# talha-alam/ADAM-Dehaze

Hardware: AMD Instinct MI355X
Metric: images/sec CORUN-Complex fwd+bwd 512x1024 bs=8; PSNR vs CPU ref (higher is better)
Workload: dtype f32; 1 GPU; CORUN-Complex (HighIntensityDehazeModel base 96) train-mode fwd + L1 + bwd + Adam; per_gpu_batch=8, global_batch=8, height=512, width=1024, parallelism=dp1

## Files before the change

adam-dehaze_amd/csrc/bn_act.hip:

```cpp
#include "common.h"

__global__ __launch_bounds__(1024) void bn_finalize_kernel(const float* __restrict__ partials, int nblk, int NcP, int C,
                                                           double count, const float* __restrict__ gamma,
                                                           const float* __restrict__ beta, float eps, float momentum,
                                                           float* running_mean, float* running_var, float* scale,
                                                           float* shift, float* save_mean, float* save_invstd, int64_t* num_batches_tracked) {
    __shared__ double red[2][32][33];
    int c;
    double S, Q, mean, var;
    if (!bn_column_sums<4>(partials, nblk, NcP, C, red, c, S, Q)) return;
    bn_mean_var(S, Q, count, mean, var);
    bn_fold_channel(c, mean, var, count, gamma, beta, eps, momentum, running_mean, running_var, scale, shift, save_mean,
                    save_invstd, num_batches_tracked);
}

extern "C" int adh_bn_finalize(void* stream, const float* partials, int nblk, int NcP, int C, double count,
                               const float* gamma, const float* beta, float eps, float momentum, float* running_mean,
                               float* running_var, float* scale, float* shift, float* save_mean, float* save_invstd,
                               int64_t* num_batches_tracked) {
    if (!partials || !scale || !shift || nblk < 1 || C < 1 || NcP < C || count <= 0) return ADH_E_ARG;
    hipLaunchKernelGGL(bn_finalize_kernel, dim3(adh_ceil_div(C, 32)), dim3(1024), 0, (hipStream_t)stream, partials, nblk,
                       NcP, C, count, gamma, beta, eps, momentum, running_mean, running_var, scale, shift, save_mean,
                       save_invstd, num_batches_tracked);
    return adh_check_launch();
}

__global__ __launch_bounds__(1024) void bn_partial_sums_kernel(const float* __restrict__ partials, int nblk, int pitch, int C,
                                                               double count, double* __restrict__ sums) {
    __shared__ double red[2][32][33];
    int c;
    double S, Q;
    if (bn_column_sums<2>(partials, nblk, pitch, C, red, c, S, Q)) {
        sums[c] = S;
        sums[C + c] = Q;
    }
    if (blockIdx.x == 0 && threadIdx.x == 0) sums[2 * C] = count;
}

extern "C" int adh_bn_partial_sums(void* stream, const float* partials, int nblk, int pitch, int C, double count, double* sums) {
    if (!partials || !sums || nblk < 1 || C < 1 || pitch < C || count <= 0) return ADH_E_ARG;
    hipLaunchKernelGGL(bn_partial_sums_kernel, dim3(adh_ceil_div(C, 32)), dim3(1024), 0, (hipStream_t)stream, partials, nblk,
                       pitch, C, count, sums);
    return adh_check_launch();
}

__global__ void bn_finalize_sums_kernel(const double* __restrict__ sums, int C, const float* __restrict__ gamma,
                                        const float* __restrict__ beta, float eps, float momentum, float* running_mean,
                                        float* running_var, float* scale, float* shift, float* save_mean, float* save_invstd,
                                        int64_t* num_batches_tracked) {
    const int c = blockIdx.x * blockDim.x + threadIdx.x;
    if (c >= C) return;
    const double count = sums[2 * C];
    double mean, var;
    bn_mean_var(sums[c], sums[C + c], count, mean, var);
    bn_fold_channel(c, mean, var, count, gamma, beta, eps, momentum, running_mean, running_var, scale, shift, save_mean,
                    save_invstd, num_batches_tracked);
}

extern "C" int adh_bn_finalize_sums(void* stream, const double* sums, int C, const float* gamma, const float* beta, float eps,
                                    float momentum, float* running_mean, float* running_var, float* scale, float* shift,
                                    float* save_mean, float* save_invstd, int64_t* num_batches_tracked) {
    if (!sums || !scale || !shift || C < 1) return ADH_E_ARG;
    hipLaunchKernelGGL(bn_finalize_sums_kernel, dim3(adh_ceil_div(C, 128)), dim3(128), 0, (hipStream_t)stream, sums, C, gamma,
                       beta, eps, momentum, running_mean, running_var, scale, shift, save_mean, save_invstd, num_batches_tracked);
    return adh_check_launch();
// ... 156 lines not shown
                    const f32x4 gg = bn_masked_grad(g[u], act, mask_bits != nullptr, mb[u], mask_ss != nullptr, yy[u], msc, msh, o[u]);
                    sg += gg;
                    sgx += gg * ((yy[u] - mu) * is);
                }
            }
        }
    }
    bn_block_fold(red, sg, sgx, CQ, R, c, C, partials);
  }
}

extern "C" int adh_bn_bwd_reduce(void* stream, const float* g_out, int g_cs, const float* out, int out_cs, int act,
                                 const float* y, int y_cs, const float* mean, const float* invstd, float* partials,
                                 int64_t P, int C, const float* mask_ss, const uint8_t* mask_bits) {
    if (!g_out || !y || !mean || !invstd || !partials || P < 1 || C < 4 || (C & 3) || C > 4096) return ADH_E_ARG;
    if (act == ADH_ACT_RELU && !out && !mask_ss && !mask_bits) return ADH_E_ARG;
    if (mask_bits && (((C / 4) & 1) || act != ADH_ACT_RELU)) return ADH_E_ARG;
    if (!adh_act_host_valid(act) || (act > ADH_ACT_RELU && !mask_ss)) return ADH_E_ARG;
    hipLaunchKernelGGL(bn_bwd_reduce_kernel, dim3(adh_bn_bwd_num_blocks(P, C)), dim3(256), 0, (hipStream_t)stream, g_out,
                       g_cs, out, out_cs, act, y, y_cs, mean, invstd, partials, P, C, mask_ss, mask_bits);
    return adh_check_launch();
}

__global__ __launch_bounds__(1024) void bn_bwd_finalize_kernel(const float* __restrict__ partials, int nblk, int pitch, int C,
                                                               double count, const float* gamma, const float* invstd,
                                                               float* dgamma, float* dbeta, int accumulate, float* coef,
                                                               int centered) {
    __shared__ double red[2][32][33];
    int c;
    double S, Q;
    if (!bn_column_sums<4>(partials, nblk, pitch, C, red, c, S, Q)) return;
    if (centered) Q *= (double)invstd[c];
    bn_bwd_coef_channel(c, C, S, Q, S, Q, count, gamma, invstd, dgamma, dbeta, accumulate, coef);
}

extern "C" int adh_bn_bwd_finalize(void* stream, const float* partials, int nblk, int C, double count,
                                   const float* gamma, const float* invstd, float* dgamma, float* dbeta, int accumulate,
                                   float* coef) {
    if (!partials || !invstd || !coef || nblk < 1 || C < 1 || count <= 0) return ADH_E_ARG;
    hipLaunchKernelGGL(bn_bwd_finalize_kernel, dim3(adh_ceil_div(C, 32)), dim3(1024), 0, (hipStream_t)stream, partials,
                       nblk, C, C, count, gamma, invstd, dgamma, dbeta, accumulate, coef, 0);
    return adh_check_launch();
}

extern "C" int adh_bn_bwd_finalize_centered(void* stream, const float* partials, int nblk, int pitch, int C, double count,
                                            const float* gamma, const float* invstd, float* dgamma, float* dbeta,
                                            int accumulate, float* coef) {
    if (!partials || !invstd || !coef || nblk < 1 || C < 1 || pitch < C || count <= 0) return ADH_E_ARG;
    hipLaunchKernelGGL(bn_bwd_finalize_kernel, dim3(adh_ceil_div(C, 32)), dim3(1024), 0, (hipStream_t)stream, partials,
                       nblk, pitch, C, count, gamma, invstd, dgamma, dbeta, accumulate, coef, 1);
    return adh_check_launch();
}

__global__ __launch_bounds__(256) void bn_bwd_apply_kernel(const float* __restrict__ g_out, int g_cs,
                                                           const float* __restrict__ out, int out_cs, int act,
                                                           const float* __restrict__ y, int y_cs,
                                                           const float* __restrict__ mean,
                                                           const float* __restrict__ invstd,
                                                           const float* __restrict__ coef, int training,
                                                           float* __restrict__ g_y, int gy_cs, float* __restrict__ g_res,
                                                           int gres_cs, int64_t P, int C, const float* __restrict__ mask_ss,
                                                           const uint8_t* __restrict__ mask_bits) {
    const int CQ = C / 4;
    int64_t p, pstep;
    int c;
    adh_stream_decode(CQ, p, pstep, c);
    const f32x4 k0 = *reinterpret_cast<const f32x4*>(coef + c);
    f32x4 mg = {0.f, 0.f, 0.f, 0.f}, kx = mg, mu = mg, msc = mg, msh = mg;
    if (mask_ss) {
        msc = *reinterpret_cast<const f32x4*>(mask_ss + c);
        msh = *reinterpret_cast<const f32x4*>(mask_ss + C + c);
    }
    if (training) {
// ... 60 lines not shown
```

adam-dehaze_amd/csrc/bn_stream.h:

```cpp
#pragma once

__host__ __device__ static inline bool adh_act_valid(int act) {
    return act == ADH_ACT_NONE || act == ADH_ACT_RELU || act == ADH_ACT_RELU6 || act == ADH_ACT_HARDSWISH ||
           act == ADH_ACT_HARDSIGMOID;
}
static inline bool adh_act_host_valid(int act) { return adh_act_valid(act); }
__device__ __forceinline__ float adh_act_fwd(int act, float z) {
    switch (act) {
        case ADH_ACT_RELU: return fmaxf(z, 0.f);
        case ADH_ACT_RELU6: return fminf(fmaxf(z, 0.f), 6.f);
        case ADH_ACT_HARDSWISH: return z * fminf(fmaxf(z + 3.f, 0.f), 6.f) / 6.f;
        case ADH_ACT_HARDSIGMOID: return fminf(fmaxf(z + 3.f, 0.f), 6.f) / 6.f;
        default: return z;
    }
}
__device__ __forceinline__ float adh_act_bwd(int act, float z, float g) {
    switch (act) {
        case ADH_ACT_RELU: return z > 0.f ? g : 0.f;
        case ADH_ACT_RELU6: return (z > 0.f && z < 6.f) ? g : 0.f;
        case ADH_ACT_HARDSWISH: return z <= -3.f ? 0.f : (z < 3.f ? g * (z / 3.f + 0.5f) : g);
        case ADH_ACT_HARDSIGMOID: return (z > -3.f && z < 3.f) ? g / 6.f : 0.f;
        default: return g;
    }
}
// ... 37 lines not shown
    CQ = (C - cbase < 1024 ? C - cbase : 1024) / 4;
    R = 256 / CQ;
    const int cq = threadIdx.x % CQ;
    prow = threadIdx.x / CQ;
    c = cbase + cq * 4;
}
__device__ __forceinline__ void bn_block_fold(f32x4 (&red)[2][256], const f32x4& a, const f32x4& b, int CQ, int R, int c, int C,
                                              float* partials) {
    red[0][threadIdx.x] = a;
    red[1][threadIdx.x] = b;
    __syncthreads();
    if (threadIdx.x < CQ) {
        f32x4 sa = {0.f, 0.f, 0.f, 0.f}, sb = {0.f, 0.f, 0.f, 0.f};
        for (int r = 0; r < R; ++r) {
            sa += red[0][r * CQ + threadIdx.x];
            sb += red[1][r * CQ + threadIdx.x];
        }
        *reinterpret_cast<f32x4*>(partials + ((size_t)blockIdx.x * 2 + 0) * C + c) = sa;
        *reinterpret_cast<f32x4*>(partials + ((size_t)blockIdx.x * 2 + 1) * C + c) = sb;
    }
    __syncthreads();
}

template <int CHAINS>
__device__ __forceinline__ bool bn_column_sums(const float* __restrict__ partials, int nblk, int pitch, int C,
                                               double (&red)[2][32][33], int& c, double& S, double& Q) {
    static_assert(CHAINS == 2 || CHAINS == 4, "two or four chains");
    const int cx = threadIdx.x & 31, ry = threadIdx.x >> 5;
    c = blockIdx.x * 32 + cx;
    double s[CHAINS] = {}, q[CHAINS] = {};
    if (c < C) {
        int b = ry;
        for (; b + 32 * (CHAINS - 1) < nblk; b += 32 * CHAINS) {
#pragma unroll
            for (int k = 0; k < CHAINS; ++k) {
                s[k] += (double)partials[((size_t)(b + 32 * k) * 2 + 0) * pitch + c];
                q[k] += (double)partials[((size_t)(b + 32 * k) * 2 + 1) * pitch + c];
            }
        }
        for (; b < nblk; b += 32) {
            s[0] += (double)partials[((size_t)b * 2 + 0) * pitch + c];
            q[0] += (double)partials[((size_t)b * 2 + 1) * pitch + c];
        }
    }
    if constexpr (CHAINS == 4) {
        red[0][ry][cx] = (s[0] + s[1]) + (s[2] + s[3]);
        red[1][ry][cx] = (q[0] + q[1]) + (q[2] + q[3]);
    } else {
        red[0][ry][cx] = s[0] + s[1];
        red[1][ry][cx] = q[0] + q[1];
    }
    __syncthreads();
    if (ry != 0 || c >= C) return false;
    S = 0.0;
    Q = 0.0;
    for (int r = 0; r < 32; ++r) {
        S += red[0][r][cx];
        Q += red[1][r][cx];
    }
    return true;
}

__device__ __forceinline__ void bn_mean_var(double S, double Q, double count, double& mean, double& var) {
    mean = S / count;
    var = Q / count - mean * mean;
    if (var < 0.0) var = 0.0;
}

__device__ __forceinline__ void bn_fold_channel(int c, double mean, double var, double count, const float* __restrict__ gamma,
                                                const float* __restrict__ beta, float eps, float momentum, float* running_mean,
                                                float* running_var, float* scale, float* shift, float* save_mean,
                                                float* save_invstd, int64_t* num_batches_tracked) {
    const double invstd = 1.0 / sqrt(var + (double)eps);
    const float gm = gamma ? gamma[c] : 1.f;
    const float bt = beta ? beta[c] : 0.f;
    scale[c] = (float)(gm * invstd);
    shift[c] = (float)(bt - mean * gm * invstd);
    if (save_mean) save_mean[c] = (float)mean;
    if (save_invstd) save_invstd[c] = (float)invstd;
    if (running_mean) running_mean[c] = (1.f - momentum) * running_mean[c] + momentum * (float)mean;
    if (running_var) {
// ... 16 lines not shown
```

adam-dehaze_amd/csrc/cbam.hip:

```cpp
#include "common.h"

#ifndef POOL_PPB
#define POOL_PPB 512
#endif
#ifndef CBAM_SCALE_MAXBLK
#define CBAM_SCALE_MAXBLK 65536
#endif
#ifndef CBAM_ROW_MAXBLK
#define CBAM_ROW_MAXBLK 2048
#endif

extern "C" int adh_cbam_pool_num_blocks(int HW) { return adh_ceil_div(HW, POOL_PPB); }

__global__ __launch_bounds__(256) void cbam_pool_partial_kernel(const float* __restrict__ x, int x_cs, int HW, int C,
                                                                float* __restrict__ partial,
                                                                int32_t* __restrict__ partial_idx, int nblk) {
    __shared__ f32x4 rs[256];
    __shared__ f32x4 rm[256];
    __shared__ int ri[256][4];
    const int n = blockIdx.y, blk = blockIdx.x;
    const int CQ = C / 4;
    const int R = 256 / CQ;
    const int cq = threadIdx.x % CQ, prow = threadIdx.x / CQ;
    const int c = cq * 4;
// ... 300 lines not shown
                            __builtin_nontemporal_load(reinterpret_cast<const f32x4*>(gn + (size_t)p * g_cs + q * 4));
            s += (v[0] + v[1]) + (v[2] + v[3]);
        }
#pragma unroll
        for (int o = 4; o > 0; o >>= 1) s += __shfl_xor(s, o, 64);
        if (sub == 0) {
            const float a = sa[(size_t)n * HW + p];
            gsa_pre[(size_t)n * HW + p] = s * a * (1.f - a);
        }
    }
}

extern "C" int adh_cbam_bwd_a(void* stream, const float* g, int g_cs, const float* x, int x_cs, const float* ca,
                              const float* sa, int N, int HW, int C, float* gsa_pre) {
    if (!g || !x || !ca || !sa || !gsa_pre || N < 1 || HW < 1 || C < 4 || (C & 3)) return ADH_E_ARG;
    const int blocks = adh_min_i(adh_ceil_div(HW, 32), CBAM_ROW_MAXBLK);
    hipLaunchKernelGGL(cbam_bwd_a_kernel, dim3(blocks, N), dim3(256), 0, (hipStream_t)stream, g, g_cs, x, x_cs, ca, sa, HW,
                       C, gsa_pre);
    return adh_check_launch();
}

extern "C" int adh_cbam_bwd_b_num_blocks(int N, int H, int W) { return adh_ceil_div((int64_t)N * H * W, 256); }

__global__ __launch_bounds__(256) void cbam_bwd_b_kernel(const float* __restrict__ gsa_pre,
                                                         const float* __restrict__ smap, const float* __restrict__ wsp,
                                                         int N, int H, int W, float* __restrict__ gsmap,
                                                         float* __restrict__ dwsp_partial) {
    __shared__ float s_w[98];
    __shared__ float s_acc[4][98];
    if (threadIdx.x < 98) s_w[threadIdx.x] = wsp[threadIdx.x];
    __syncthreads();
    const int64_t total = (int64_t)N * H * W;
    const int64_t idx = (int64_t)blockIdx.x * 256 + threadIdx.x;
    const bool valid = idx < total;
    int n = 0, y = 0, xx = 0;
    if (valid) {
        xx = (int)(idx % W);
        const int64_t r = idx / W;
        y = (int)(r % H);
        n = (int)(r / H);
    }
    const float* gp = gsa_pre + (size_t)n * H * W;
    const float* sm = smap + (size_t)n * H * W * 2;
    const float gs_here = valid ? gp[(size_t)y * W + xx] : 0.f;
    float g0 = 0.f, g1 = 0.f;
    const int wave = threadIdx.x >> 6, lane = threadIdx.x & 63;
    for (int ky = 0; ky < 7; ++ky) {
        for (int kx = 0; kx < 7; ++kx) {
            const int oy = y - ky + 3, ox = xx - kx + 3;
            if (valid && oy >= 0 && oy < H && ox >= 0 && ox < W) {
                const float go = gp[(size_t)oy * W + ox];
                g0 += go * s_w[ky * 7 + kx];
                g1 += go * s_w[49 + ky * 7 + kx];
            }
            const int iy = y + ky - 3, ix = xx + kx - 3;
            float a0 = 0.f, a1 = 0.f;
            if (valid && iy >= 0 && iy < H && ix >= 0 && ix < W) {
                const float* q = sm + ((size_t)iy * W + ix) * 2;
                a0 = q[0] * gs_here;
                a1 = q[1] * gs_here;
            }
            a0 = wave_sum(a0);
            a1 = wave_sum(a1);
            if (lane == 0) {
                s_acc[wave][ky * 7 + kx] = a0;
                s_acc[wave][49 + ky * 7 + kx] = a1;
            }
        }
    }
    if (valid) {
        gsmap[idx * 2 + 0] = g0;
        gsmap[idx * 2 + 1] = g1;
    }
    __syncthreads();
    if (threadIdx.x < 98)
        dwsp_partial[(size_t)blockIdx.x * 98 + threadIdx.x] =
            (s_acc[0][threadIdx.x] + s_acc[1][threadIdx.x]) + (s_acc[2][threadIdx.x] + s_acc[3][threadIdx.x]);
}

__global__ __launch_bounds__(256) void cbam_dwsp_final_kernel(const float* __restrict__ partial, int nblk, float* dwsp,
                                                              int accumulate) {
    __shared__ double red[256];
    const int o = blockIdx.x;
    double s = 0.0;
    for (int b = threadIdx.x; b < nblk; b += 256) s += (double)partial[(size_t)b * 98 + o];
    red[threadIdx.x] = s;
    __syncthreads();
    for (int st = 128; st > 0; st >>= 1) {
        if (threadIdx.x < st) red[threadIdx.x] += red[threadIdx.x + st];
        __syncthreads();
    }
    if (threadIdx.x == 0) dwsp[o] = accumulate ? dwsp[o] + (float)red[0] : (float)red[0];
}

extern "C" int adh_cbam_bwd_b(void* stream, const float* gsa_pre, const float* smap, const float* wsp, int N, int H,
                              int W, float* gsmap, float* dwsp_partial, int nblk, float* dwsp, int accumulate) {
    if (!gsa_pre || !smap || !wsp || !gsmap || !dwsp_partial || !dwsp) return ADH_E_ARG;
    if (nblk != adh_cbam_bwd_b_num_blocks(N, H, W)) return ADH_E_ARG;
    hipStream_t s = (hipStream_t)stream;
    hipLaunchKernelGGL(cbam_bwd_b_kernel, dim3(nblk), dim3(256), 0, s, gsa_pre, smap, wsp, N, H, W, gsmap, dwsp_partial);
// ... 226 lines not shown
```

adam-dehaze_amd/csrc/conv_wgrad.hip:

```cpp
#include "common.h"
#include <cstdlib>

#define WG_TW 32

template <int T, int TN>
__global__ __launch_bounds__(512, 2) void conv_wgrad_kernel(const adh_conv_desc d, const ConvGeom g, float* slab,
                                                            int ntiles, int KP, int nco_groups) {
    extern __shared__ __attribute__((aligned(16))) float smem[];
    constexpr int BN = 32 * TN;
    constexpr int PER = (T * TN + 3) / 4;
    const int XP = g.xp;
    const int buf_floats = g.npx * XP + 32 + g.TH * WG_TW * BN;

    const int tid = threadIdx.x;
    const int lane = tid & 63;
    const int wave = __builtin_amdgcn_readfirstlane(tid >> 6);
    const bool loader = wave >= 4;
    const int l31 = lane & 31;
    const int h = lane >> 5;

    const int ci_tile = blockIdx.x / nco_groups;
    const int co_grp = blockIdx.x - ci_tile * nco_groups;
    const int ci0 = ci_tile * 32;
    const int co0 = co_grp * BN;
// ... 456 lines not shown
        if (2 * bytes <= 160 * 1024 || TH == 1) break;
        TH >>= 1;
    }
    g->TH = TH;
    g->npxp = g->npx;
    g->tiles_x = adh_ceil_div(d->VW, WG_TW);
    g->tiles_y = adh_ceil_div(d->VH, TH);
    g->KC = 32;
    g->KQ_log2 = 3;
    g->KQtot = 0;
    g->xp = xp;
    return ADH_OK;
}

template <int T, int TN>
static void launch_wgrad(hipStream_t s, const adh_conv_desc* d, const ConvGeom& g, float* slab, int nsplit, int KP) {
    const int ntiles = g.tiles_x * g.tiles_y * d->N;
    const int nco_groups = d->NcP / (32 * TN);
    const int lds = 2 * (g.npx * g.xp * 4 + 128 + g.TH * WG_TW * 32 * TN * 4);
    dim3 grid((KP / 32) * nco_groups, nsplit, (d->KH * d->KW) / T);
    (void)hipFuncSetAttribute(reinterpret_cast<const void*>(&conv_wgrad_kernel<T, TN>),
                              hipFuncAttributeMaxDynamicSharedMemorySize, 160 * 1024);
    hipLaunchKernelGGL((conv_wgrad_kernel<T, TN>), grid, dim3(512), lds, s, *d, g, slab, ntiles, KP, nco_groups);
}

static int wgrad_pick_tn(int NcP, int T) {
    const int t = NcP / 32;
    for (int tn = 4; tn >= 1; --tn)
        if (t % tn == 0 && (T * tn + 3) / 4 <= 12) return tn;
    return 1;
}

struct WrPlan {
    int KH, KW, rev, TN;
    WrArgs a;
};

static int wgrad_rows_plan(const adh_conv_desc* d, int nsplit, WrPlan plan[4]) {
    if (d->VW % 32 != 0 || d->VH % WR_TH != 0) return 0;
    if (d->Cin % 32 != 0 || d->Cout % 4 != 0 || d->NcP != adh_round_up(d->Cout, 32)) return 0;
    if (d->in_cstride % 4 != 0 || d->out_cstride % 4 != 0) return 0;
    if (d->in_sy != d->in_sx || d->dstep_y != d->dstep_x || d->out_sy != d->out_sx) return 0;
    if ((d->VH - 1) * d->out_sy + d->out_oy >= d->OH || (d->VW - 1) * d->out_sx + d->out_ox >= d->OW) return 0;
    if ((int64_t)(d->IH + 8) * d->IW * d->in_cstride * 4 >= (int64_t)1 << 31) return 0;
    if ((int64_t)d->OH * d->OW * d->out_cstride * 4 >= (int64_t)1 << 31) return 0;
    const int t = d->NcP / 32;
// ... 113 lines not shown
        WrPlan plan[4];
        const int np = wgrad_rows_plan(d, nsplit, plan);
        if (np && wgrad_rows_instantiated(plan[0])) {
            for (int i = 0; i < np; ++i) {
                const int rc = dispatch_wgrad_rows((hipStream_t)stream, d, plan[i], slab);
                if (rc) return rc;
            }
            return ADH_OK;
        }
    }
    const int Ttot = d->KH * d->KW;
    int T;
    if (Ttot == 9 || Ttot == 16 || Ttot == 4 || Ttot == 1) T = Ttot;
    else if (Ttot == 49 || Ttot == 14) T = 7;
    else return ADH_E_UNSUPPORTED;
    const bool packed = (d->dstep_x == 4 && d->Cin == 8 && d->in_sx == 1);
    const int TN = wgrad_pick_tn(d->NcP, T);
    ConvGeom g;
    int rc = wgrad_geometry(d, &g, TN, packed ? 8 : 32);
    if (rc) return rc;
    if ((d->VH - 1) * d->out_sy + d->out_oy >= d->OH || (d->VW - 1) * d->out_sx + d->out_ox >= d->OW) return ADH_E_ARG;
    const int KP = adh_round_up(d->Cin, 32);
    hipStream_t s = (hipStream_t)stream;
#define WG_CASE(t, tn) \
    if (T == t && TN == tn) { launch_wgrad<t, tn>(s, d, g, slab, nsplit, KP); return adh_check_launch(); }
    WG_CASE(9, 4) WG_CASE(9, 3) WG_CASE(9, 2) WG_CASE(9, 1)
    WG_CASE(16, 3) WG_CASE(16, 2) WG_CASE(16, 1)
    WG_CASE(4, 4) WG_CASE(4, 3) WG_CASE(4, 2) WG_CASE(4, 1)
    WG_CASE(7, 4) WG_CASE(7, 3) WG_CASE(7, 2) WG_CASE(7, 1)
    WG_CASE(1, 4) WG_CASE(1, 3) WG_CASE(1, 2) WG_CASE(1, 1)
#undef WG_CASE
    return ADH_E_UNSUPPORTED;
}
```

adam-dehaze_amd/csrc/conv_wgrad_small.hip:

```cpp
#include "common.h"

typedef float f32x4s __attribute__((ext_vector_type(4)));

template <int XC, int GC, int CIB>
__global__ __launch_bounds__(256) void conv_wgrad_small_kernel(const adh_conv_desc d, int tiles_x, int tiles_y, int ntiles,
                                                               float* __restrict__ slab, int KP, int NcP) {
    extern __shared__ __attribute__((aligned(16))) float lds[];
    constexpr int XS_F = 6 * 66 * XC + 16;
    float* const xs = lds;
    float* const gs = lds + XS_F;

    const int tid = threadIdx.x;
    const int lane = tid & 63;
    const int wave = tid >> 6;
    const int i16 = lane & 15, kk = lane >> 4;

    f32x4s acc[9 * CIB];
#pragma unroll
    for (int t = 0; t < 9 * CIB; ++t) acc[t] = f32x4s{0.f, 0.f, 0.f, 0.f};

    for (int tile = blockIdx.x; tile < ntiles; tile += gridDim.x) {
        int r = tile;
        const int tx = r % tiles_x;
        r /= tiles_x;
        const int ty = r % tiles_y;
        const int n = r / tiles_y;
        const int y0 = ty * 4, x0 = tx * 64;
        const float* xin = d.in + (int64_t)n * d.IH * d.IW * XC;
        const float* gin = d.out + (int64_t)n * d.VH * d.VW * GC;
        __syncthreads();
        constexpr int XQ = XC / 4;
        for (int i = tid; i < 6 * 66 * XQ; i += 256) {
            const int px = i / XQ, q = i - px * XQ;
            const int row = px / 66, col = px - row * 66;
            const int iy = y0 - 1 + row, ix = x0 - 1 + col;
            f32x4s v = {0.f, 0.f, 0.f, 0.f};
            if (iy >= 0 && iy < d.IH && ix >= 0 && ix < d.IW)
                v = *reinterpret_cast<const f32x4s*>(xin + ((int64_t)iy * d.IW + ix) * XC + q * 4);
            *reinterpret_cast<f32x4s*>(xs + px * XC + q * 4) = v;
        }
        constexpr int GQ = GC / 4;
        for (int i = tid; i < 4 * 64 * GQ; i += 256) {
            const int px = i / GQ, q = i - px * GQ;
            const int row = px >> 6, col = px & 63;
            const int gy = y0 + row, gx = x0 + col;
            f32x4s v = {0.f, 0.f, 0.f, 0.f};
            if (gy < d.VH && gx < d.VW) v = *reinterpret_cast<const f32x4s*>(gin + ((int64_t)gy * d.VW + gx) * GC + q * 4);
            *reinterpret_cast<f32x4s*>(gs + px * GC + q * 4) = v;
        }
        if (tid < 16) {
            xs[6 * 66 * XC + tid] = 0.f;
            gs[4 * 64 * GC + tid] = 0.f;
        }
        __syncthreads();
        const float* gl = gs + (wave * 64 + kk) * GC + i16;
        const float* xl = xs + (wave * 66 + kk) * XC + i16;
#pragma unroll 2
        for (int kg = 0; kg < 16; ++kg) {
            const float b = gl[kg * 4 * GC];
#pragma unroll
            for (int dy = 0; dy < 3; ++dy)
#pragma unroll
                for (int dx = 0; dx < 3; ++dx)
#pragma unroll
                    for (int cb = 0; cb < CIB; ++cb) {
                        const float a = xl[(dy * 66 + kg * 4 + dx) * XC + cb * 16];
                        acc[(dy * 3 + dx) * CIB + cb] =
                            __builtin_amdgcn_mfma_f32_16x16x4f32(a, b, acc[(dy * 3 + dx) * CIB + cb], 0, 0, 0);
                    }
        }
    }

    float* red = lds;
#pragma unroll 1
    for (int w = 1; w < 4; ++w) {
        __syncthreads();
        if (wave == w) {
// ... 26 lines not shown
                                                                float* __restrict__ slab, int KP, int NcP) {
    extern __shared__ __attribute__((aligned(16))) float lds[];
    constexpr int CJB = XC / 16;
    constexpr int RT = (9 * COUT + 15) / 16;
    constexpr int GS_F = 6 * 66 * GC + 16;
    float* const gs = lds;
    float* const xs = lds + GS_F;
    const int tid = threadIdx.x;
    const int lane = tid & 63;
    const int wave = tid >> 6;
    const int i16 = lane & 15, kk = lane >> 4;
    int aoff[RT];
#pragma unroll
    for (int t = 0; t < RT; ++t) {
        const int rI = adh_min_i(t * 16 + i16, 9 * COUT - 1);
        const int tap = rI / COUT, co = rI - tap * COUT;
        const int dy = tap / 3, dx = tap - dy * 3;
        aoff[t] = ((2 - dy) * 66 + (2 - dx)) * GC + co;
    }
    f32x4s acc[RT * CJB];
#pragma unroll
    for (int t = 0; t < RT * CJB; ++t) acc[t] = f32x4s{0.f, 0.f, 0.f, 0.f};

    for (int tile = blockIdx.x; tile < ntiles; tile += gridDim.x) {
        int r = tile;
        const int tx = r % tiles_x;
        r /= tiles_x;
        const int ty = r % tiles_y;
        const int n = r / tiles_y;
        const int y0 = ty * 4, x0 = tx * 64;
        const float* xin = d.in + (int64_t)n * d.IH * d.IW * XC;
        const float* gin = d.out + (int64_t)n * d.VH * d.VW * GC;
        __syncthreads();
        constexpr int GQ = GC / 4;
        for (int i = tid; i < 6 * 66 * GQ; i += 256) {
            const int px = i / GQ, q = i - px * GQ;
            const int row = px / 66, col = px - row * 66;
            const int gy = y0 - 1 + row, gx = x0 - 1 + col;
            f32x4s v = {0.f, 0.f, 0.f, 0.f};
            if (gy >= 0 && gy < d.VH && gx >= 0 && gx < d.VW) v = *reinterpret_cast<const f32x4s*>(gin + ((int64_t)gy * d.VW + gx) * GC + q * 4);
            *reinterpret_cast<f32x4s*>(gs + px * GC + q * 4) = v;
        }
        constexpr int XQ = XC / 4;
        for (int i = tid; i < 4 * 64 * XQ; i += 256) {
            const int px = i / XQ, q = i - px * XQ;
            const int row = px >> 6, col = px & 63;
            const int iy = y0 + row, ix = x0 + col;
            f32x4s v = {0.f, 0.f, 0.f, 0.f};
            if (iy < d.IH && ix < d.IW) v = *reinterpret_cast<const f32x4s*>(xin + ((int64_t)iy * d.IW + ix) * XC + q * 4);
            *reinterpret_cast<f32x4s*>(xs + px * XC + q * 4) = v;
        }
        if (tid < 16) gs[6 * 66 * GC + tid] = 0.f;
        __syncthreads();
        const float* gl = gs + (wave * 66 + kk) * GC;
        const float* xl = xs + (wave * 64 + kk) * XC + i16;
#pragma unroll 4
        for (int kg = 0; kg < 16; ++kg) {
            float a[RT], b[CJB];
#pragma unroll
            for (int t = 0; t < RT; ++t) a[t] = gl[kg * 4 * GC + aoff[t]];
#pragma unroll
            for (int c = 0; c < CJB; ++c) b[c] = xl[kg * 4 * XC + c * 16];
#pragma unroll
            for (int t = 0; t < RT; ++t)
#pragma unroll
                for (int c = 0; c < CJB; ++c)
                    acc[t * CJB + c] = __builtin_amdgcn_mfma_f32_16x16x4f32(a[t], b[c], acc[t * CJB + c], 0, 0, 0);
        }
    }
    float* red = lds;
#pragma unroll 1
    for (int w = 1; w < 4; ++w) {
        __syncthreads();
        if (wave == w) {
#pragma unroll
            for (int t = 0; t < RT * CJB; ++t) *reinterpret_cast<f32x4s*>(red + (t * 64 + lane) * 4) = acc[t];
// ... 71 lines not shown
```

adam-dehaze_amd/csrc/densenet.hip:

```cpp
#include "common.h"

#define SS_PPB 512
#define SS_UNROLL 4

extern "C" int adh_bn_slice_stats_num_blocks(int64_t P, int C) {
    (void)C;
    return P < 1 ? ADH_E_ARG : adh_ceil_div(P, SS_PPB);
}

__global__ __launch_bounds__(256) void bn_slice_stats_kernel(const float* __restrict__ x, int x_cs, int64_t P, int C,
                                                             float* __restrict__ partials) {
    __shared__ f32x4 red[2][256];
    for (int cbase = 0; cbase < C; cbase += 1024) {
        int CQ, R, prow, c;
        bn_group_decode(C, cbase, CQ, R, prow, c);
        f32x4 s = {0.f, 0.f, 0.f, 0.f}, q = s;
        if (prow < R) {
            const int64_t p0 = (int64_t)blockIdx.x * SS_PPB;
            const int64_t p1 = p0 + SS_PPB < P ? p0 + SS_PPB : P;
            for (int64_t p = p0 + prow; p < p1; p += SS_UNROLL * R) {
                f32x4 v[SS_UNROLL];
#pragma unroll
                for (int u = 0; u < SS_UNROLL; ++u) {
                    const int64_t r = p + u * R < p1 ? p + u * R : p;
                    v[u] = __builtin_nontemporal_load(reinterpret_cast<const f32x4*>(x + r * x_cs + c));
                }
#pragma unroll
                for (int u = 0; u < SS_UNROLL; ++u)
                    if (p + u * R < p1) {
                        s += v[u];
                        q += v[u] * v[u];
                    }
            }
        }
        bn_block_fold(red, s, q, CQ, R, c, C, partials);
    }
}

extern "C" int adh_bn_slice_stats(void* stream, const float* x, int x_cs, int64_t P, int C, float* partials) {
    if (!x || !partials || P < 1 || C < 4 || (C & 3) || C > 4096 || x_cs < C || (x_cs & 3)) return ADH_E_ARG;
    hipLaunchKernelGGL(bn_slice_stats_kernel, dim3(adh_bn_slice_stats_num_blocks(P, C)), dim3(256), 0, (hipStream_t)stream, x,
                       x_cs, P, C, partials);
    return adh_check_launch();
}

__global__ __launch_bounds__(1024) void bn_slice_moments_kernel(const float* __restrict__ partials, int nblk, int pitch, int C,
                                                                double count, double* __restrict__ mean,
                                                                double* __restrict__ var) {
    __shared__ double red[2][32][33];
    int c;
    double S, Q, m, v;
    if (!bn_column_sums<2>(partials, nblk, pitch, C, red, c, S, Q)) return;
    bn_mean_var(S, Q, count, m, v);
    mean[c] = m;
    var[c] = v;
}

extern "C" int adh_bn_slice_moments(void* stream, const float* partials, int nblk, int pitch, int C, double count, double* mean,
                                    double* var) {
    if (!partials || !mean || !var || nblk < 1 || C < 1 || pitch < C || count <= 0) return ADH_E_ARG;
    hipLaunchKernelGGL(bn_slice_moments_kernel, dim3(adh_ceil_div(C, 32)), dim3(1024), 0, (hipStream_t)stream, partials, nblk,
                       pitch, C, count, mean, var);
    return adh_check_launch();
}

__global__ void bn_fold_moments_kernel(int C, const double* __restrict__ mean, const double* __restrict__ var, double count,
                                       const float* __restrict__ gamma, const float* __restrict__ beta, float eps,
                                       float momentum, float* running_mean, float* running_var, float* scale, float* shift,
                                       float* save_mean, float* save_invstd, int64_t* num_batches_tracked) {
    const int c = blockIdx.x * blockDim.x + threadIdx.x;
    if (c >= C) return;
    bn_fold_channel(c, mean[c], var[c], count, gamma, beta, eps, momentum, running_mean, running_var, scale, shift, save_mean,
                    save_invstd, num_batches_tracked);
}

extern "C" int adh_bn_fold_moments(void* stream, int C, const double* mean, const double* var, double count, const float* gamma,
                                   const float* beta, float eps, float momentum, float* running_mean, float* running_var,
                                   float* scale, float* shift, float* save_mean, float* save_invstd,
                                   int64_t* num_batches_tracked) {
    if (C < 1 || !mean || !var || !scale || !shift || count <= 0) return ADH_E_ARG;
    hipLaunchKernelGGL(bn_fold_moments_kernel, dim3(adh_ceil_div(C, 256)), dim3(256), 0, (hipStream_t)stream, C, mean, var, count,
                       gamma, beta, eps, momentum, running_mean, running_var, scale, shift, save_mean, save_invstd,
                       num_batches_tracked);
    return adh_check_launch();
}
// ... 87 lines not shown
```

Baseline: 40.43 images/sec.

## Retune BN column reduction, prefetch wgrad tiles, add 1x1 few-output wgrad kernel

BN column-sum kernels now use 8 channels per block with 256 threads and a batched, unrolled load loop, which gives more blocks and more loads in flight per thread. The small-channel wgrad kernels prefetch the next tile into registers while computing the current one, overlapping global loads with compute at the cost of extra registers. A dedicated 1x1 wgrad kernel handles layers with at most 32 inputs and 4 outputs. The CBAM backward replaces per-tap wave reductions with LDS staging and a per-row fold, which adds shared memory and barriers.

New measurement: 40.68 images/sec (median of 6 runs). No clear change (+0.6%).

```diff
diff --git a/adam-dehaze_amd/csrc/bn_act.hip b/adam-dehaze_amd/csrc/bn_act.hip
--- a/adam-dehaze_amd/csrc/bn_act.hip
+++ b/adam-dehaze_amd/csrc/bn_act.hip
@@ -1,11 +1,12 @@
 #include "common.h"
 
-__global__ __launch_bounds__(1024) void bn_finalize_kernel(const float* __restrict__ partials, int nblk, int NcP, int C,
+__global__ __launch_bounds__(BN_COLS_THREADS) void bn_finalize_kernel(const float* __restrict__ partials,
+                                                                    int nblk, int NcP, int C,
                                                            double count, const float* __restrict__ gamma,
                                                            const float* __restrict__ beta, float eps, float momentum,
                                                            float* running_mean, float* running_var, float* scale,
                                                            float* shift, float* save_mean, float* save_invstd, int64_t* num_batches_tracked) {
-    __shared__ double red[2][32][33];
+    __shared__ BnColsLds red;
     int c;
     double S, Q, mean, var;
     if (!bn_column_sums<4>(partials, nblk, NcP, C, red, c, S, Q)) return;
@@ -19,15 +20,16 @@
                                float* running_var, float* scale, float* shift, float* save_mean, float* save_invstd,
                                int64_t* num_batches_tracked) {
     if (!partials || !scale || !shift || nblk < 1 || C < 1 || NcP < C || count <= 0) return ADH_E_ARG;
-    hipLaunchKernelGGL(bn_finalize_kernel, dim3(adh_ceil_div(C, 32)), dim3(1024), 0, (hipStream_t)stream, partials, nblk,
-                       NcP, C, count, gamma, beta, eps, momentum, running_mean, running_var, scale, shift, save_mean,
-                       save_invstd, num_batches_tracked);
-    return adh_check_launch();
-}
-
-__global__ __launch_bounds__(1024) void bn_partial_sums_kernel(const float* __restrict__ partials, int nblk, int pitch, int C,
+    hipLaunchKernelGGL(bn_finalize_kernel, dim3(adh_ceil_div(C, BN_COLS_CH)), dim3(BN_COLS_THREADS), 0, (hipStream_t)stream,
+                       partials, nblk, NcP, C, count, gamma, beta, eps, momentum, running_mean, running_var, scale, shift,
+                       save_mean, save_invstd, num_batches_tracked);
+    return adh_check_launch();
+}
+
+__global__ __launch_bounds__(BN_COLS_THREADS) void bn_partial_sums_kernel(const float* __restrict__ partials,
+                                                                        int nblk, int pitch, int C,
                                                                double count, double* __restrict__ sums) {
-    __shared__ double red[2][32][33];
+    __shared__ BnColsLds red;
     int c;
     double S, Q;
     if (bn_column_sums<2>(partials, nblk, pitch, C, red, c, S, Q)) {
@@ -39,8 +41,8 @@
 
 extern "C" int adh_bn_partial_sums(void* stream, const float* partials, int nblk, int pitch, int C, double count, double* sums) {
     if (!partials || !sums || nblk < 1 || C < 1 || pitch < C || count <= 0) return ADH_E_ARG;
-    hipLaunchKernelGGL(bn_partial_sums_kernel, dim3(adh_ceil_div(C, 32)), dim3(1024), 0, (hipStream_t)stream, partials, nblk,
-                       pitch, C, count, sums);
+    hipLaunchKernelGGL(bn_partial_sums_kernel, dim3(adh_ceil_div(C, BN_COLS_CH)), dim3(BN_COLS_THREADS), 0, (hipStream_t)stream,
+                       partials, nblk, pitch, C, count, sums);
     return adh_check_launch();
 }
 
@@ -243,11 +245,12 @@
     return adh_check_launch();
 }
 
-__global__ __launch_bounds__(1024) void bn_bwd_finalize_kernel(const float* __restrict__ partials, int nblk, int pitch, int C,
+__global__ __launch_bounds__(BN_COLS_THREADS) void bn_bwd_finalize_kernel(const float* __restrict__ partials,
+                                                                        int nblk, int pitch, int C,
                                                                double count, const float* gamma, const float* invstd,
                                                                float* dgamma, float* dbeta, int accumulate, float* coef,
                                                                int centered) {
-    __shared__ double red[2][32][33];
+    __shared__ BnColsLds red;
     int c;
     double S, Q;
     if (!bn_column_sums<4>(partials, nblk, pitch, C, red, c, S, Q)) return;
@@ -259,8 +262,8 @@
                                    const float* gamma, const float* invstd, float* dgamma, float* dbeta, int accumulate,
                                    float* coef) {
     if (!partials || !invstd || !coef || nblk < 1 || C < 1 || count <= 0) return ADH_E_ARG;
-    hipLaunchKernelGGL(bn_bwd_finalize_kernel, dim3(adh_ceil_div(C, 32)), dim3(1024), 0, (hipStream_t)stream, partials,
-                       nblk, C, C, count, gamma, invstd, dgamma, dbeta, accumulate, coef, 0);
+    hipLaunchKernelGGL(bn_bwd_finalize_kernel, dim3(adh_ceil_div(C, BN_COLS_CH)), dim3(BN_COLS_THREADS), 0, (hipStream_t)stream,
+                       partials, nblk, C, C, count, gamma, invstd, dgamma, dbeta, accumulate, coef, 0);
     return adh_check_launch();
 }
 
@@ -268,8 +271,8 @@
                                             const float* gamma, const float* invstd, float* dgamma, float* dbeta,
                                             int accumulate, float* coef) {
     if (!partials || !invstd || !coef || nblk < 1 || C < 1 || pitch < C || count <= 0) return ADH_E_ARG;
-    hipLaunchKernelGGL(bn_bwd_finalize_kernel, dim3(adh_ceil_div(C, 32)), dim3(1024), 0, (hipStream_t)stream, partials,
-                       nblk, pitch, C, count, gamma, invstd, dgamma, dbeta, accumulate, coef, 1);
+    hipLaunchKernelGGL(bn_bwd_finalize_kernel, dim3(adh_ceil_div(C, BN_COLS_CH)), dim3(BN_COLS_THREADS), 0, (hipStream_t)stream,
+                       partials, nblk, pitch, C, count, gamma, invstd, dgamma, dbeta, accumulate, coef, 1);
     return adh_check_launch();
 }
 
diff --git a/adam-dehaze_amd/csrc/bn_stream.h b/adam-dehaze_amd/csrc/bn_stream.h
--- a/adam-dehaze_amd/csrc/bn_stream.h
+++ b/adam-dehaze_amd/csrc/bn_stream.h
@@ -83,15 +83,46 @@
     __syncthreads();
 }
 
+#define BN_COLS_CH 8
+#define BN_COLS_U 32
+#define BN_COLS_THREADS (32 * BN_COLS_CH)
+struct BnColsLds {
+    double v[2][32][BN_COLS_CH + 1];
+};
+template <int CHAINS, int U>
+__device__ __forceinline__ void bn_column_batch(const float* __restrict__ col, int pitch, int b, double (&s)[CHAINS],
+                                                double (&q)[CHAINS]) {
+    float vs[U][CHAINS], vq[U][CHAINS];
+#pragma unroll
+    for (int u = 0; u < U; ++u) {
+#pragma unroll
+        for (int k = 0; k < CHAINS; ++k) {
+            const float* row = col + (size_t)(b + 32 * (u * CHAINS + k)) * 2 * pitch;
+            vs[u][k] = row[0];
+            vq[u][k] = row[pitch];
+        }
+    }
+#pragma unroll
+    for (int u = 0; u < U; ++u) {
+#pragma unroll
+        for (int k = 0; k < CHAINS; ++k) {
+            s[k] += (double)vs[u][k];
+            q[k] += (double)vq[u][k];
+        }
+    }
+}
 template <int CHAINS>
 __device__ __forceinline__ bool bn_column_sums(const float* __restrict__ partials, int nblk, int pitch, int C,
-                                               double (&red)[2][32][33], int& c, double& S, double& Q) {
+                                               BnColsLds& red, int& c, double& S, double& Q) {
     static_assert(CHAINS == 2 || CHAINS == 4, "two or four chains");
-    const int cx = threadIdx.x & 31, ry = threadIdx.x >> 5;
-    c = blockIdx.x * 32 + cx;
+    const int cx = threadIdx.x % BN_COLS_CH, ry = threadIdx.x / BN_COLS_CH;
+    c = blockIdx.x * BN_COLS_CH + cx;
     double s[CHAINS] = {}, q[CHAINS] = {};
     if (c < C) {
         int b = ry;
+        for (; b + 32 * (BN_COLS_U - 1) < nblk; b += 32 * BN_COLS_U)
+            bn_column_batch<CHAINS, BN_COLS_U / CHAINS>(partials + c, pitch, b, s, q);
+        for (; b + 32 * 7 < nblk; b += 32 * 8) bn_column_batch<CHAINS, 8 / CHAINS>(partials + c, pitch, b, s, q);
         for (; b + 32 * (CHAINS - 1) < nblk; b += 32 * CHAINS) {
 #pragma unroll
             for (int k = 0; k < CHAINS; ++k) {
@@ -105,19 +136,19 @@
         }
     }
     if constexpr (CHAINS == 4) {
-        red[0][ry][cx] = (s[0] + s[1]) + (s[2] + s[3]);
-        red[1][ry][cx] = (q[0] + q[1]) + (q[2] + q[3]);
+        red.v[0][ry][cx] = (s[0] + s[1]) + (s[2] + s[3]);
+        red.v[1][ry][cx] = (q[0] + q[1]) + (q[2] + q[3]);
     } else {
-        red[0][ry][cx] = s[0] + s[1];
-        red[1][ry][cx] = q[0] + q[1];
+        red.v[0][ry][cx] = s[0] + s[1];
+        red.v[1][ry][cx] = q[0] + q[1];
     }
     __syncthreads();
     if (ry != 0 || c >= C) return false;
     S = 0.0;
     Q = 0.0;
     for (int r = 0; r < 32; ++r) {
-        S += red[0][r][cx];
-        Q += red[1][r][cx];
+        S += red.v[0][r][cx];
+        Q += red.v[1][r][cx];
     }
     return true;
 }
diff --git a/adam-dehaze_amd/csrc/cbam.hip b/adam-dehaze_amd/csrc/cbam.hip
--- a/adam-dehaze_amd/csrc/cbam.hip
+++ b/adam-dehaze_amd/csrc/cbam.hip
@@ -346,12 +346,42 @@
 
 extern "C" int adh_cbam_bwd_b_num_blocks(int N, int H, int W) { return adh_ceil_div((int64_t)N * H * W, 256); }
 
+#define CBAM_B_PROD_Q (14 * 256 / 4)
+#define CBAM_B_PART_Q (98 * 4 * 8 / 4)
+__device__ __forceinline__ int cbam_b_slot() {
+    const int wave = threadIdx.x >> 6, lane = threadIdx.x & 63;
+    return wave * 64 + (lane & 7) * 8 + (lane >> 3);
+}
+__device__ __forceinline__ void cbam_b_fold_row(const f32x4* s_prod, f32x4* s_part, int ky) {
+    float* part = reinterpret_cast<float*>(s_part);
+    __syncthreads();
+    for (int it = threadIdx.x; it < 14 * 4 * 8; it += 256) {
+        const f32x4 lo = s_prod[it * 2], hi = s_prod[it * 2 + 1];
+        const int ch = it / (7 * 32), r = it - ch * (7 * 32);
+        part[(ch * 49 + ky * 7) * 32 + r] = ((lo[0] + hi[0]) + (lo[2] + hi[2])) + ((lo[1] + hi[1]) + (lo[3] + hi[3]));
+    }
+    __syncthreads();
+}
+__device__ __forceinline__ void cbam_b_rows(const f32x4* s_part, float* __restrict__ dwsp_partial) {
+    if (threadIdx.x < 98) {
+        float sw[4];
+#pragma unroll
+        for (int w = 0; w < 4; ++w) {
+            const f32x4 lo = s_part[(threadIdx.x * 4 + w) * 2], hi = s_part[(threadIdx.x * 4 + w) * 2 + 1];
+            sw[w] = ((lo[0] + hi[0]) + (lo[2] + hi[2])) + ((lo[1] + hi[1]) + (lo[3] + hi[3]));
+        }
+        dwsp_partial[(size_t)blockIdx.x * 98 + threadIdx.x] = (sw[0] + sw[1]) + (sw[2] + sw[3]);
+    }
+}
+
 __global__ __launch_bounds__(256) void cbam_bwd_b_kernel(const float* __restrict__ gsa_pre,
                                                          const float* __restrict__ smap, const float* __restrict__ wsp,
                                                          int N, int H, int W, float* __restrict__ gsmap,
                                                          float* __restrict__ dwsp_partial) {
     __shared__ float s_w[98];
-    __shared__ float s_acc[4][98];
+    __shared__ f32x4 s_prod[CBAM_B_PROD_Q];
+    __shared__ f32x4 s_part[CBAM_B_PART_Q];
+    float* prod = reinterpret_cast<float*>(s_prod);
     if (threadIdx.x < 98) s_w[threadIdx.x] = wsp[threadIdx.x];
     __syncthreads();
     const int64_t total = (int64_t)N * H * W;
@@ -368,7 +398,7 @@
     const float* sm = smap + (size_t)n * H * W * 2;
     const float gs_here = valid ? gp[(size_t)y * W + xx] : 0.f;
     float g0 = 0.f, g1 = 0.f;
-    const int wave = threadIdx.x >> 6, lane = threadIdx.x & 63;
+    const int slot = cbam_b_slot();
     for (int ky = 0; ky < 7; ++ky) {
         for (int kx = 0; kx < 7; ++kx) {
             const int oy = y - ky + 3, ox = xx - kx + 3;
@@ -384,22 +414,16 @@
                 a0 = q[0] * gs_here;
                 a1 = q[1] * gs_here;
             }
-            a0 = wave_sum(a0);
-            a1 = wave_sum(a1);
-            if (lane == 0) {
-                s_acc[wave][ky * 7 + kx] = a0;
-                s_acc[wave][49 + ky * 7 + kx] = a1;
-            }
-        }
+            prod[kx * 256 + slot] = a0;
+            prod[(7 + kx) * 256 + slot] = a1;
+        }
+        cbam_b_fold_row(s_prod, s_part, ky);
     }
     if (valid) {
         gsmap[idx * 2 + 0] = g0;
         gsmap[idx * 2 + 1] = g1;
     }
-    __syncthreads();
-    if (threadIdx.x < 98)
-        dwsp_partial[(size_t)blockIdx.x * 98 + threadIdx.x] =
-            (s_acc[0][threadIdx.x] + s_acc[1][threadIdx.x]) + (s_acc[2][threadIdx.x] + s_acc[3][threadIdx.x]);
+    cbam_b_rows(s_part, dwsp_partial);
 }
 
 __global__ __launch_bounds__(256) void cbam_dwsp_final_kernel(const float* __restrict__ partial, int nblk, float* dwsp,
diff --git a/adam-dehaze_amd/csrc/conv_wgrad.hip b/adam-dehaze_amd/csrc/conv_wgrad.hip
--- a/adam-dehaze_amd/csrc/conv_wgrad.hip
+++ b/adam-dehaze_amd/csrc/conv_wgrad.hip
@@ -502,6 +502,71 @@
     (void)hipFuncSetAttribute(reinterpret_cast<const void*>(&conv_wgrad_kernel<T, TN>),
                               hipFuncAttributeMaxDynamicSharedMemorySize, 160 * 1024);
     hipLaunchKernelGGL((conv_wgrad_kernel<T, TN>), grid, dim3(512), lds, s, *d, g, slab, ntiles, KP, nco_groups);
+}
+
+#define W1_U 8
+__global__ __launch_bounds__(256) void conv_wgrad_1x1_fewout_kernel(const adh_conv_desc d, int CQ, float* __restrict__ slab, int KP) {
+    __shared__ float red[256][17];
+    __shared__ float fin[32][4];
+    const int PL = 256 / CQ;
+    const int pl = threadIdx.x / CQ, q = threadIdx.x - pl * CQ;
+    const int P = d.N * d.VH * d.VW;
+    const int step = gridDim.x * PL;
+    float acc[16];
+#pragma unroll
+    for (int e = 0; e < 16; ++e) acc[e] = 0.f;
+    if (pl < PL) {
+        for (int64_t p0 = (int64_t)blockIdx.x * PL + pl; p0 < P; p0 += (int64_t)step * W1_U) {
+            f32x4 xv[W1_U], gv[W1_U];
+#pragma unroll
+            for (int u = 0; u < W1_U; ++u) {
+                const int64_t p64 = p0 + (int64_t)u * step;
+                const bool inside = p64 < P;
+                const unsigned p = inside ? (unsigned)p64 : 0u;
+                const unsigned row = p / (unsigned)d.VW, vx = p - row * (unsigned)d.VW;
+                const unsigned n = row / (unsigned)d.VH, vy = row - n * (unsigned)d.VH;
+                const int iy = (int)vy * d.in_sy + d.dy0, ix = (int)vx * d.in_sx + d.dx0;
+                const bool okx = inside && iy >= 0 && iy < d.IH && ix >= 0 && ix < d.IW;
+                const float* xs = okx ? d.in + (((size_t)n * d.IH + iy) * d.IW + ix) * d.in_cstride + q * 4 : d.in;
+                const int oy = (int)vy * d.out_sy + d.out_oy, ox = (int)vx * d.out_sx + d.out_ox;
+                const float* gs = d.out + (((size_t)n * d.OH + oy) * d.OW + ox) * d.out_cstride;
+                xv[u] = *reinterpret_cast<const f32x4*>(xs);
+                gv[u] = *reinterpret_cast<const f32x4*>(gs);
+                if (!okx) xv[u] = f32x4{0.f, 0.f, 0.f, 0.f};
+                if (!inside) gv[u] = f32x4{0.f, 0.f, 0.f, 0.f};
+            }
+#pragma unroll
+            for (int u = 0; u < W1_U; ++u)
+#pragma unroll
+                for (int i = 0; i < 4; ++i)
+#pragma unroll
+                    for (int j = 0; j < 4; ++j) acc[i * 4 + j] = fmaf(xv[u][i], gv[u][j], acc[i * 4 + j]);
+        }
+    }
+#pragma unroll
+    for (int e = 0; e < 16; ++e) red[threadIdx.x][e] = acc[e];
+    if (threadIdx.x < 128) fin[threadIdx.x >> 2][threadIdx.x & 3] = 0.f;
+    __syncthreads();
+    if ((int)threadIdx.x < CQ * 16) {
+        const int q2 = threadIdx.x >> 4, e = threadIdx.x & 15;
+        float s = 0.f;
+        for (int l = 0; l < PL; ++l) s += red[l * CQ + q2][e];
+        const int ci = q2 * 4 + (e >> 2), co = e & 3;
+        if (ci < d.Cin && co < d.Cout) fin[ci][co] = s;
+    }
+    __syncthreads();
+    float* sl = slab + (size_t)blockIdx.x * KP * d.NcP;
+    for (int i = threadIdx.x; i < KP * d.NcP; i += 256) {
+        const int ci = i / d.NcP, co = i - ci * d.NcP;
+        sl[i] = (ci < 32 && co < 4) ? fin[ci][co] : 0.f;
+    }
+}
+
+static bool wgrad_1x1_fewout_ok(const adh_conv_desc* d) {
+    if (d->KH != 1 || d->KW != 1 || d->Cin < 1 || d->Cin > 32 || d->Cout < 1 || d->Cout > 4) return false;
+    if (d->in_cstride % 4 != 0 || d->out_cstride % 4 != 0 || d->Cin > d->in_cstride || d->Cout > d->out_cstride) return false;
+    if (((uintptr_t)d->in & 15) || ((uintptr_t)d->out & 15)) return false;
+    return (int64_t)d->N * d->VH * d->VW < ((int64_t)1 << 31) - 1;
 }
 
 static int wgrad_pick_tn(int NcP, int T) {
@@ -661,6 +726,10 @@
     if ((d->VH - 1) * d->out_sy + d->out_oy >= d->OH || (d->VW - 1) * d->out_sx + d->out_ox >= d->OW) return ADH_E_ARG;
     const int KP = adh_round_up(d->Cin, 32);
     hipStream_t s = (hipStream_t)stream;
+    if (wgrad_1x1_fewout_ok(d)) {
+        hipLaunchKernelGGL(conv_wgrad_1x1_fewout_kernel, dim3(nsplit), dim3(256), 0, s, *d, (d->Cin + 3) / 4, slab, KP);
+        return adh_check_launch();
+    }
 #define WG_CASE(t, tn) \
     if (T == t && TN == tn) { launch_wgrad<t, tn>(s, d, g, slab, nsplit, KP); return adh_check_launch(); }
     WG_CASE(9, 4) WG_CASE(9, 3) WG_CASE(9, 2) WG_CASE(9, 1)
diff --git a/adam-dehaze_amd/csrc/conv_wgrad_small.hip b/adam-dehaze_amd/csrc/conv_wgrad_small.hip
--- a/adam-dehaze_amd/csrc/conv_wgrad_small.hip
+++ b/adam-dehaze_amd/csrc/conv_wgrad_small.hip
@@ -1,6 +1,46 @@
 #include "common.h"
 
 typedef float f32x4s __attribute__((ext_vector_type(4)));
+
+template <int C, int R, int CN>
+struct WgsTile {
+    static constexpr int Q = C / 4, TOTAL = R * CN * Q, NL = (TOTAL + 255) / 256;
+};
+template <int C, int R, int CN>
+__device__ __forceinline__ void wgs_fetch(const float* __restrict__ img, int H, int W, int oy, int ox,
+                                          f32x4s (&v)[WgsTile<C, R, CN>::NL]) {
+    using T = WgsTile<C, R, CN>;
+#pragma unroll
+    for (int l = 0; l < T::NL; ++l) {
+        const int i = threadIdx.x + l * 256;
+        f32x4s t = {0.f, 0.f, 0.f, 0.f};
+        if (i < T::TOTAL) {
+            const int px = i / T::Q, q = i - px * T::Q;
+            const int row = px / CN, col = px - row * CN;
+            const int iy = oy + row, ix = ox + col;
+            if (iy >= 0 && iy < H && ix >= 0 && ix < W)
+                t = *reinterpret_cast<const f32x4s*>(img + ((int64_t)iy * W + ix) * C + q * 4);
+        }
+        v[l] = t;
+    }
+}
+template <int C, int R, int CN>
+__device__ __forceinline__ void wgs_stash(float* tile, const f32x4s (&v)[WgsTile<C, R, CN>::NL]) {
+    using T = WgsTile<C, R, CN>;
+#pragma unroll
+    for (int l = 0; l < T::NL; ++l) {
+        const int i = threadIdx.x + l * 256;
+        if (i < T::TOTAL) *reinterpret_cast<f32x4s*>(tile + i * 4) = v[l];
+    }
+}
+__device__ __forceinline__ void wgs_decode(int tile, int tiles_x, int tiles_y, int& n, int& y0, int& x0) {
+    const int tx = tile % tiles_x;
+    tile /= tiles_x;
+    const int ty = tile % tiles_y;
+    n = tile / tiles_y;
+    y0 = ty * 4;
+    x0 = tx * 64;
+}
 
 template <int XC, int GC, int CIB>
 __global__ __launch_bounds__(256) void conv_wgrad_small_kernel(const adh_conv_desc d, int tiles_x, int tiles_y, int ntiles,
@@ -19,40 +59,24 @@
 #pragma unroll
     for (int t = 0; t < 9 * CIB; ++t) acc[t] = f32x4s{0.f, 0.f, 0.f, 0.f};
 
+    f32x4s xr[WgsTile<XC, 6, 66>::NL], gr[WgsTile<GC, 4, 64>::NL];
+    auto fetch = [&](int tile) {
+        int n, y0, x0;
+        wgs_decode(tile, tiles_x, tiles_y, n, y0, x0);
+        wgs_fetch<XC, 6, 66>(d.in + (int64_t)n * d.IH * d.IW * XC, d.IH, d.IW, y0 - 1, x0 - 1, xr);
+        wgs_fetch<GC, 4, 64>(d.out + (int64_t)n * d.VH * d.VW * GC, d.VH, d.VW, y0, x0, gr);
+    };
+    fetch(blockIdx.x);
+    if (tid < 16) {
+        xs[6 * 66 * XC + tid] = 0.f;
+        gs[4 * 64 * GC + tid] = 0.f;
+    }
     for (int tile = blockIdx.x; tile < ntiles; tile += gridDim.x) {
-        int r = tile;
-        const int tx = r % tiles_x;
-        r /= tiles_x;
-        const int ty = r % tiles_y;
-        const int n = r / tiles_y;
-        const int y0 = ty * 4, x0 = tx * 64;
-        const float* xin = d.in + (int64_t)n * d.IH * d.IW * XC;
-        const float* gin = d.out + (int64_t)n * d.VH * d.VW * GC;
-        __syncthreads();
-        constexpr int XQ = XC / 4;
-        for (int i = tid; i < 6 * 66 * XQ; i += 256) {
-            const int px = i / XQ, q = i - px * XQ;
-            const int row = px / 66, col = px - row * 66;
-            const int iy = y0 - 1 + row, ix = x0 - 1 + col;
-            f32x4s v = {0.f, 0.f, 0.f, 0.f};
-            if (iy >= 0 && iy < d.IH && ix >= 0 && ix < d.IW)
-                v = *reinterpret_cast<const f32x4s*>(xin + ((int64_t)iy * d.IW + ix) * XC + q * 4);
-            *reinterpret_cast<f32x4s*>(xs + px * XC + q * 4) = v;
-        }
-        constexpr int GQ = GC / 4;
-        for (int i = tid; i < 4 * 64 * GQ; i += 256) {
-            const int px = i / GQ, q = i - px * GQ;
-            const int row = px >> 6, col = px & 63;
-            const int gy = y0 + row, gx = x0 + col;
-            f32x4s v = {0.f, 0.f, 0.f, 0.f};
-            if (gy < d.VH && gx < d.VW) v = *reinterpret_cast<const f32x4s*>(gin + ((int64_t)gy * d.VW + gx) * GC + q * 4);
-            *reinterpret_cast<f32x4s*>(gs + px * GC + q * 4) = v;
-        }
-        if (tid < 16) {
-            xs[6 * 66 * XC + tid] = 0.f;
-            gs[4 * 64 * GC + tid] = 0.f;
-        }
-        __syncthreads();
+        __syncthreads();
+        wgs_stash<XC, 6, 66>(xs, xr);
+        wgs_stash<GC, 4, 64>(gs, gr);
+        __syncthreads();
+        if (tile + (int)gridDim.x < ntiles) fetch(tile + gridDim.x);
         const float* gl = gs + (wave * 64 + kk) * GC + i16;
         const float* xl = xs + (wave * 66 + kk) * XC + i16;
 #pragma unroll 2
@@ -125,36 +149,21 @@
 #pragma unroll
     for (int t = 0; t < RT * CJB; ++t) acc[t] = f32x4s{0.f, 0.f, 0.f, 0.f};
 
+    f32x4s gr[WgsTile<GC, 6, 66>::NL], xr[WgsTile<XC, 4, 64>::NL];
+    auto fetch = [&](int tile) {
+        int n, y0, x0;
+        wgs_decode(tile, tiles_x, tiles_y, n, y0, x0);
+        wgs_fetch<GC, 6, 66>(d.out + (int64_t)n * d.VH * d.VW * GC, d.VH, d.VW, y0 - 1, x0 - 1, gr);
+        wgs_fetch<XC, 4, 64>(d.in + (int64_t)n * d.IH * d.IW * XC, d.IH, d.IW, y0, x0, xr);
+    };
+    fetch(blockIdx.x);
+    if (tid < 16) gs[6 * 66 * GC + tid] = 0.f;
     for (int tile = blockIdx.x; tile < ntiles; tile += gridDim.x) {
-        int r = tile;
-        const int tx = r % tiles_x;
-        r /= tiles_x;
-        const int ty = r % tiles_y;
-        const int n = r / tiles_y;
-        const int y0 = ty * 4, x0 = tx * 64;
-        const float* xin = d.in + (int64_t)n * d.IH * d.IW * XC;
-        const float* gin = d.out + (int64_t)n * d.VH * d.VW * GC;
-        __syncthreads();
-        constexpr int GQ = GC / 4;
-        for (int i = tid; i < 6 * 66 * GQ; i += 256) {
-            const int px = i / GQ, q = i - px * GQ;
-            const int row = px / 66, col = px - row * 66;
-            const int gy = y0 - 1 + row, gx = x0 - 1 + col;
-            f32x4s v = {0.f, 0.f, 0.f, 0.f};
-            if (gy >= 0 && gy < d.VH && gx >= 0 && gx < d.VW) v = *reinterpret_cast<const f32x4s*>(gin + ((int64_t)gy * d.VW + gx) * GC + q * 4);
-            *reinterpret_cast<f32x4s*>(gs + px * GC + q * 4) = v;
-        }
-        constexpr int XQ = XC / 4;
-        for (int i = tid; i < 4 * 64 * XQ; i += 256) {
-            const int px = i / XQ, q = i - px * XQ;
-            const int row = px >> 6, col = px & 63;
-            const int iy = y0 + row, ix = x0 + col;
-            f32x4s v = {0.f, 0.f, 0.f, 0.f};
-            if (iy < d.IH && ix < d.IW) v = *reinterpret_cast<const f32x4s*>(xin + ((int64_t)iy * d.IW + ix) * XC + q * 4);
-            *reinterpret_cast<f32x4s*>(xs + px * XC + q * 4) = v;
-        }
-        if (tid < 16) gs[6 * 66 * GC + tid] = 0.f;
-        __syncthreads();
+        __syncthreads();
+        wgs_stash<GC, 6, 66>(gs, gr);
+        wgs_stash<XC, 4, 64>(xs, xr);
+        __syncthreads();
+        if (tile + (int)gridDim.x < ntiles) fetch(tile + gridDim.x);
         const float* gl = gs + (wave * 66 + kk) * GC;
         const float* xl = xs + (wave * 64 + kk) * XC + i16;
 #pragma unroll 4
diff --git a/adam-dehaze_amd/csrc/densenet.hip b/adam-dehaze_amd/csrc/densenet.hip
--- a/adam-dehaze_amd/csrc/densenet.hip
+++ b/adam-dehaze_amd/csrc/densenet.hip
@@ -44,10 +44,11 @@
     return adh_check_launch();
 }
 
-__global__ __launch_bounds__(1024) void bn_slice_moments_kernel(const float* __restrict__ partials, int nblk, int pitch, int C,
+__global__ __launch_bounds__(BN_COLS_THREADS) void bn_slice_moments_kernel(const float* __restrict__ partials,
+                                                                         int nblk, int pitch, int C,
                                                                 double count, double* __restrict__ mean,
                                                                 double* __restrict__ var) {
-    __shared__ double red[2][32][33];
+    __shared__ BnColsLds red;
     int c;
     double S, Q, m, v;
     if (!bn_column_sums<2>(partials, nblk, pitch, C, red, c, S, Q)) return;
@@ -59,8 +60,8 @@
 extern "C" int adh_bn_slice_moments(void* stream, const float* partials, int nblk, int pitch, int C, double count, double* mean,
                                     double* var) {
     if (!partials || !mean || !var || nblk < 1 || C < 1 || pitch < C || count <= 0) return ADH_E_ARG;
-    hipLaunchKernelGGL(bn_slice_moments_kernel, dim3(adh_ceil_div(C, 32)), dim3(1024), 0, (hipStream_t)stream, partials, nblk,
-                       pitch, C, count, mean, var);
+    hipLaunchKernelGGL(bn_slice_moments_kernel, dim3(adh_ceil_div(C, BN_COLS_CH)), dim3(BN_COLS_THREADS), 0, (hipStream_t)stream,
+                       partials, nblk, pitch, C, count, mean, var);
     return adh_check_launch();
 }
 
```
